# Project-MONAI/GenerativeModels

Hardware: AMD Instinct MI355X
Metric: 3D volumes/sec (DDIM 50-step sample, 1x128^3) (higher is better)
Workload: dtype bf16; 1 GPU; C2: 3D DiffusionModelUNet(64,128,256; 2 res blocks; mid-block attention 1 head x 256) DDIM-50 sampling of 1x1x128^3 volumes, 1 volume per GPU per step; inference_steps=50, parallelism=1 independent replicas (batch-sharded, no data-path collective), hip_graph=False, self_launched=False

## Files before the change

### generativemodels_amd/csrc/conv_dma.hip

```cpp
#include "conv_dma_shared.h"
#include <type_traits>

#ifdef GM_CONV_TIMELINE
#define TL_STAMP(k)                                                                                                              \
  do {                                                                                                                           \
    if ((p.debug_flags & 4096) && threadIdx.x == 0 && tl_on)                                                                            \
      reinterpret_cast<unsigned long long*>(p.kpartial)[(long long)blockIdx.x * 64 + (k)] = __builtin_readcyclecounter();        \
  } while (0)
#else
#define TL_STAMP(k)
#endif
#ifndef GM_DMA_PART
#define GM_DMA_PART (-1)
#endif
#define DMA_PART(k) (GM_DMA_PART == -1 || GM_DMA_PART == (k))
static __device__ __attribute__((aligned(64))) unsigned int gm_zero_row[16] = {0};

template <typename T, int NW, int MF, int S, int MINW, int KS = 3, int NFR_ = 4, bool PRE = false>
__global__ __launch_bounds__(64 * NW, MINW) void conv_dma_kernel(const GmConvDesc p, const unsigned phase_wgs, const unsigned phase_sleeps) {
  constexpr int BK = ConvTraits<T>::BK;
  constexpr int VECW = ConvTraits<T>::VECW;
  constexpr int NT = 64 * NW;
  constexpr int NFR = NFR_, G = KS == 3 ? 3 : 2, RING = KS == 3 ? 3 : 4;
  static_assert(KS == 3 || (KS == 2 && S == 1 && (NW == 8 || NW == 4)), "the sub-pixel variant is stride 1, 8 waves x 32 or 4 waves x 64 voxels");
  static_assert(NW * MF * 16 == 512 || NW * MF * 16 == (S == 1 ? 256 : 128), "waves x fragments cover the tile");
  constexpr int TH = 4, TW = 16, BM = NW * MF * 16, TD = BM / (TH * TW);
  constexpr int NPW = KS == 2 ? 2 : 1;
  constexpr int PD = S * (TD - 1) + KS, PH = S * (TH - 1) + KS, PW = S * (TW - 1) + KS + (NPW - 1);
  constexpr int EW = TW + 1;
  constexpr int PLANE = ((PH * PW + 15) / 16) * 16;
  constexpr int PROWS = PD * PLANE;
  constexpr int PPIECES = PROWS / 16;
  constexpr int PPW = (PPIECES + NW - 1) / NW;
  constexpr int BN = 16 * NFR;
  constexpr int WROWS = G * BN;
  constexpr bool WGEN = NFR != 4 || (KS == 2 && NW == 4);
  constexpr int PATCH_BYTES = PROWS * DMA_ROWB;
  constexpr int WBUF_BYTES = WROWS * DMA_ROWB;
  constexpr int PVT_OFF = PATCH_BYTES + (KS == 2 ? 36864 : RING * WBUF_BYTES) + 512;
  constexpr int NGROUPS = KS * KS * KS / G * NPW;
  constexpr int WPW = WGEN ? WROWS / 16 / NW : (KS == 2 ? 1 : (NW == 8 ? 2 : (NW == 4 ? 3 : 1)));
  static_assert(!WGEN || (S == 1 && (WROWS / 16) % NW == 0), "general panel distribution: whole pieces per wave");
  static_assert(WROWS == (KS == 3 ? 3 : 2) * BN, "G taps per weight panel");
  static_assert(NGROUPS % RING == 0, "the ring slot of a group is a compile-time constant");
#ifdef GM_CONV_LDS_EPILOGUE
  constexpr bool DIRECT_W = false;
#else
  constexpr bool DIRECT_W = NFR == 4 && KS == 3;
#endif

  extern __shared__ __attribute__((aligned(1024))) char smem[];
  const unsigned lds0 = (unsigned)(uintptr_t)smem;

  const int tid = threadIdx.x;
  const int lane = tid & 63;
  const int wave = __builtin_amdgcn_readfirstlane(tid >> 6);
  const int l15 = lane & 15, q = lane >> 4;
  if (blockIdx.x < phase_wgs) {
    const unsigned tg = __builtin_amdgcn_s_getreg((3 << 11) | (16 << 6) | 4);
    if (tg & 1) {
      for (unsigned k = phase_sleeps; k > 0; --k) __builtin_amdgcn_s_sleep(16);
    }
  }

  const int Dt = KS == 2 ? p.Ds : p.Do, Ht = KS == 2 ? p.Hs : p.Ho, Wt = KS == 2 ? p.Ws : p.Wo;
  const int ntd = (Dt + TD - 1) / TD, nth = (Ht + TH - 1) / TH, ntw = (Wt + TW - 1) / TW;
  const int ncb = (p.Cout + BN - 1) / BN;
  const int ksplit = (KS == 3 && S == 1 && p.kpartial && p.ksplit > 1) ? p.ksplit : 1;
  int Dv = p.Ds, Hv = p.Hs, Wv = p.Ws;
  if (p.in_mode == 1) { Dv *= p.fd; Hv *= p.fh; Wv *= p.fw; }
  const int nchunks = p.Cin / BK;
  const int cout_pad = (p.Cout + 15) & ~15;
  const int cps = ksplit > 1 ? (nchunks + ksplit - 1) / ksplit : nchunks;

  const unsigned nwork = (unsigned)p.N * ntd * nth * ntw * ncb * (KS == 2 ? 4u : 1u) * (unsigned)ksplit;
  const unsigned xcd = blockIdx.x & 7, gx = (gridDim.x >> 3) + (xcd < (gridDim.x & 7) ? 1u : 0u);
  const unsigned q8 = nwork >> 3, r8 = nwork & 7, cx = q8 + (xcd < r8 ? 1u : 0u), sx = xcd < r8 ? xcd * (q8 + 1) : r8 * (q8 + 1) + (xcd - r8) * q8;
  unsigned pos = blockIdx.x >> 3;
  if (pos >= cx) return;
#ifdef GM_CONV_TIMELINE
  const unsigned tl_pos = pos + gx < cx ? pos + gx : pos;
#endif

  struct Tile { int cb, par, n, td_i, th_i, tw_i, ks; };
  auto decode = [&](unsigned wi) __attribute__((always_inline)) {
    Tile t;
    unsigned b = wi;
    t.ks = 0;
    if (ksplit > 1) {
      const unsigned tiles_all = nwork / (unsigned)ksplit;
      t.ks = (int)(b / tiles_all);
      b -= (unsigned)t.ks * tiles_all;
    }
    t.cb = b % ncb; b /= ncb;
    t.par = 0;
    if (KS == 2) { t.par = b & 3; b >>= 2; }
    t.tw_i = b % ntw; b /= ntw;
    t.th_i = b % nth; b /= nth;
    t.td_i = b % ntd; b /= ntd;
    t.n = b;
    return t;
  };

  const char* zero = reinterpret_cast<const char*>(gm_zero_row);
  const char* xbase = reinterpret_cast<const char*>(p.x);
  int psw = 0;
#pragma unroll
  for (int j = 0; j < PPW; ++j) {
    const int row = 16 * (wave + NW * j) + (lane >> 2);
    const int rr = row % PLANE;
    psw |= dma_swz(rr % PW) << (2 * j);
  }
  int pvox[PPW];
  constexpr bool PVOX_LDS = KS == 2 && NW == 4;
  int* pvt = reinterpret_cast<int*>(smem + PVT_OFF) + threadIdx.x;
  if (PVOX_LDS) pvt[PPW * NT] = psw;
  auto place_patch = [&](const Tile& t) __attribute__((always_inline)) {
    KDesc& pk = cold_desc();
    const int ud0 = t.td_i * TD * S - (KS == 2 ? 1 - ((t.par >> 1) & 1) : pk.pd), uh0 = t.th_i * TH * S - (KS == 2 ? 1 - (t.par & 1) : pk.ph),
              uw0 = t.tw_i * TW * S - (KS == 2 ? 1 : pk.pw);
    OPAQUE_LANE(lane_p);
#pragma unroll
    for (int j = 0; j < PPW; ++j) {
      const int row = 16 * (wave + NW * j) + (lane_p >> 2);
      const int pa = row / PLANE, rr = row - pa * PLANE;
      const int pb = rr / PW, lc = rr - pb * PW;
      const int pc = S == 1 ? lc : (lc < EW ? 2 * lc : 2 * (lc - EW) + 1);
      int ud = ud0 + pa, uh = uh0 + pb, uw = uw0 + pc;
      const bool ok = (row < PROWS) & (rr < PH * PW) & (ud >= 0) & (ud < Dv) & (uh >= 0) & (uh < Hv) & (uw >= 0) & (uw < Wv);
      if (pk.in_mode == 1) { ud /= pk.fd; uh /= pk.fh; uw /= pk.fw; }
      const int pvj = ok ? ((t.n * pk.Ds + ud) * pk.Hs + uh) * pk.Ws + uw : -1;
      if (PVOX_LDS) pvt[j * NT] = pvj; else pvox[j] = pvj;
    }
  };
  const long long xrowb = p.x_ld * (long long)sizeof(T);
  const char* x2base = reinterpret_cast<const char*>(p.x2);
  const long long x2rowb = p.x2_ld * (long long)sizeof(T);
  const int nchunks0 = p.x2 ? p.cin_split / BK : nchunks;
  auto issue_patch = [&](int chunk) __attribute__((always_inline)) {
#ifdef GM_CONV_ABLATE
    if (p.debug_flags & 1024) return;
#endif
    const bool second = chunk >= nchunks0;
    const char* cbase = second ? x2base + (long long)(chunk - nchunks0) * (BK * (int)sizeof(T)) : xbase + (long long)chunk * (BK * (int)sizeof(T));
    const long long rowb = second ? x2rowb : xrowb;
#pragma unroll
    for (int j = 0; j < PPW; ++j) {
      if (wave + NW * j < PPIECES) {
        int pv = PVOX_LDS ? pvt[j * NT] : pvox[j];
        asm volatile("" : "+v"(pv));
        int ps = PVOX_LDS ? pvt[PPW * NT] : psw;
        if (PVOX_LDS) asm volatile("" : "+v"(ps));
        const char* src = pv >= 0 ? cbase + pv * rowb + (((lane & 3) ^ ((ps >> (2 * j)) & 3)) << 4) : zero + ((lane & 3) << 4);
        dma16(src, lds0 + (unsigned)(16 * (wave + NW * j)) * DMA_ROWB);
      }
    }
  };

  Tile cur = decode(sx + pos);
  const Tile stride = decode(gx);
  place_patch(cur);
  if (min(nchunks, cur.ks * cps) < nchunks) issue_patch(min(nchunks, cur.ks * cps));

  constexpr bool pre = PRE;
  float sc[VECW], sh[VECW];
  auto load_affine = [&](int chunk) __attribute__((always_inline)) {
    const int c0 = chunk * BK + (lane & 3) * VECW;
    const float* ps = p.pre_scale + (long long)cur.n * p.Cin + c0;
    const float* ph = p.pre_shift + (long long)cur.n * p.Cin + c0;
#pragma unroll
    for (int i = 0; i < VECW; i += 4) {
      const float4 a = *reinterpret_cast<const float4*>(ps + i), b = *reinterpret_cast<const float4*>(ph + i);
      sc[i] = a.x; sc[i + 1] = a.y; sc[i + 2] = a.z; sc[i + 3] = a.w;
      sh[i] = b.x; sh[i + 1] = b.y; sh[i + 2] = b.z; sh[i + 3] = b.w;
    }
  };
  auto transform_patch = [&]() __attribute__((always_inline)) {
#pragma unroll
    for (int j = 0; j < PPW; ++j) {
      if (wave + NW * j < PPIECES && pvox[j] >= 0) {
        char* a = smem + (16 * (wave + NW * j) + (lane >> 2)) * DMA_ROWB + (((lane & 3) ^ ((psw >> (2 * j)) & 3)) << 4);
        float v[VECW];
        Vec16<T>::unpack(*reinterpret_cast<const uint4*>(a), v);
#pragma unroll
        for (int i = 0; i < VECW; ++i) v[i] = v[i] * sc[i] + sh[i];
        conv_act_vec(v, p.pre_act, sizeof(T) == 4);
        *reinterpret_cast<uint4*>(a) = Vec16<T>::pack(v);
      }
    }
    asm volatile("s_waitcnt lgkmcnt(0)" ::: "memory");
  };


  const char* wbase = nullptr;
  int wsrc[WPW];
  auto place_weights = [&](const Tile& t) __attribute__((always_inline)) {
    KDesc& pk = cold_desc();
    wbase = reinterpret_cast<const char*>(pk.w) + (long long)(t.par * NPW) * nchunks * (KS * KS * KS) * cout_pad * DMA_ROWB;
    OPAQUE_LANE(lane_w);
#pragma unroll
    for (int h = 0; h < WPW; ++h) {
      const int row = WGEN ? 16 * (wave + NW * h) + (lane_w >> 2)
                    : KS == 2 ? 16 * wave + (lane_w >> 2)
                              : NW == 8 ? (h == 0 ? 16 * wave + (lane_w >> 2) : 128 + 8 * wave + ((lane_w & 31) >> 2))
                                        : (NW == 4 ? 16 * (wave + NW * h) + (lane_w >> 2) : 16 * (wave < 12 ? wave : 0) + (lane_w >> 2));
      const int u = row / BN, col = row % BN;
      const int co = t.cb * BN + (DIRECT_W ? direct_col_chan<T>(col) : col);
      wsrc[h] = co < cout_pad ? ((u * cout_pad + co) * DMA_ROWB + (((lane_w & 3) ^ dma_swz(row)) << 4)) : -1;
    }
  };
  auto issue_w_pieces = [&](int t, int buf, int h0, int h1) __attribute__((always_inline)) {
#ifdef GM_CONV_ABLATE
    if (p.debug_flags & 512) return;
#endif
    const char* panel = KS == 2 ? wbase + ((long long)((t & 7) >> 2) * nchunks * 8 + (long long)(t >> 3) * 8 + 2 * (t & 3)) * cout_pad * DMA_ROWB
                                : wbase + (long long)t * G * cout_pad * DMA_ROWB;
    const unsigned dst = lds0 + PATCH_BYTES + (unsigned)buf * WBUF_BYTES;
#pragma unroll
    for (int h = h0; h < h1; ++h) {
      const char* src = wsrc[h] >= 0 ? panel + wsrc[h] : zero + ((lane & 3) << 4);
      if (WGEN) {
        dma16(src, dst + (unsigned)(16 * (wave + NW * h)) * DMA_ROWB);
      } else if (KS == 2) {
        dma16(src, dst + (unsigned)(16 * wave) * DMA_ROWB);
      } else if (NW == 8) {
        if (h == 0) dma16(src, dst + (unsigned)(16 * wave) * DMA_ROWB);
        else if (lane < 32) dma16(src, dst + (unsigned)(128 + 8 * wave) * DMA_ROWB);
      } else if (NW == 16) {
        if (wave < 12) dma16(src, dst + (unsigned)(16 * wave) * DMA_ROWB);
      } else {
        dma16(src, dst + (unsigned)(16 * (wave + NW * h)) * DMA_ROWB);
      }
    }
  };
  auto issue_w = [&](int t, int buf) __attribute__((always_inline)) { issue_w_pieces(t, buf, 0, WPW); };


  constexpr int SCRATCH_WAVE = MF * 16 * 144, SCRATCH_BYTES = NW * SCRATCH_WAVE;
  constexpr int RING_BYTES = KS == 2 ? (RING * WBUF_BYTES > 36864 ? RING * WBUF_BYTES : 36864) : RING * WBUF_BYTES;
  constexpr bool EARLY = SCRATCH_BYTES <= RING_BYTES;
  constexpr int SCRATCH_OFF = EARLY ? PATCH_BYTES : 0;
  static_assert(EARLY || SCRATCH_BYTES <= PATCH_BYTES + RING_BYTES, "the transpose scratch fits under the addend vector");
  static_assert(BN * 8 <= SCRATCH_WAVE, "a wave's statistic partials fit into its scratch block");
  static_assert(PVT_OFF == PATCH_BYTES + RING_BYTES + 512, "the placement table follows the addend vector");
  float* addv = reinterpret_cast<float*>(smem + PATCH_BYTES + RING_BYTES);
#ifdef GM_CONV_LDS_EPILOGUE
  constexpr bool DIRECT = false;
#else
  constexpr bool DIRECT = NFR == 4 && KS == 3;
#endif
  constexpr int EPASSES = (NFR * 16 * (int)sizeof(T) + 127) / 128;
  constexpr int CH_PER_PASS = 128 / (int)sizeof(T);
  static_assert(EPASSES <= 4, "at most 4 epilogue passes (128 output channels in fp32)");

  for (;;) {
#ifdef GM_CONV_TIMELINE
    const bool tl_on = pos == tl_pos;
#endif
    TL_STAMP(0);
    const int c_begin = min(nchunks, cur.ks * cps), c_end = min(nchunks, c_begin + cps);
    const int total = (c_end - c_begin) * NGROUPS;
    const int od0 = cur.td_i * TD, oh0 = cur.th_i * TH, ow0 = cur.tw_i * TW;
    TL_STAMP(1);
    place_weights(cur);
    if (total > 0) {
      issue_w(c_begin * NGROUPS, 0);
      if (total > 1) issue_w(c_begin * NGROUPS + 1, 1);
      if (pre) load_affine(c_begin);
    }
    float addend = 0.f;
    KDesc& pa = cold_desc();
    OPAQUE_LANE(lane_a);
    const int tid_a = wave * 64 + lane_a;
    if (tid_a < BN) {
      const int co = cur.cb * BN + tid_a;
      if (co < pa.Cout) {
        if (pa.bias) addend += pa.bias[co];
        if (pa.skip_bias) addend += pa.skip_bias[co];
        if (pa.rowvec) addend += pa.rowvec[(long long)cur.n * pa.rowvec_bstride + co];
      }
    }
    TL_STAMP(55);
    constexpr int HK = S * (MF - 1) + KS;
    static_assert(MF <= 4 && (4 % MF) == 0, "a wave's fragments stay inside one 4-row tile plane");
    OPAQUE_LANE(lane_t);
    const int l15t = lane_t & 15, qt = lane_t >> 4;
    constexpr int NXA = KS + NPW - 1;
    int xa[NXA];
    {
      const int m0 = wave * MF * 16 + l15t;
      const int a = m0 >> 6, bb0 = (m0 >> 4) & 3, c = m0 & 15;
#pragma unroll
      for (int kw = 0; kw < NXA; ++kw) {
        const int col = S == 1 ? c + kw : (kw == 1 ? EW + c : c + (kw >> 1));
        xa[kw] = (S * a * PLANE + S * bb0 * PW + col) * DMA_ROWB + ((qt ^ dma_swz(col)) << 4);
      }
    }
    const int wa0 = PATCH_BYTES + l15t * DMA_ROWB + ((qt ^ dma_swz(l15t)) << 4);
#define XADDR(hk, kw) (xa[kw] + (hk) * (PW * DMA_ROWB))
#define WADDR(nf) (wa0 + (nf) * (16 * DMA_ROWB))
    f32x4_t accs[NPW][NFR][MF];
#pragma unroll
    for (int pw = 0; pw < NPW; ++pw)
#pragma unroll
      for (int nf = 0; nf < NFR; ++nf)
#pragma unroll
        for (int mf = 0; mf < MF; ++mf) accs[pw][nf][mf] = (f32x4_t){0.f, 0.f, 0.f, 0.f};
    f32x4_t (&acc)[NFR][MF] = accs[0];
    if (tid_a < BN) addv[tid_a] = addend;
    TL_STAMP(56);
    if (total > 0) {
      dma_wait<0>();
      if (pre) transform_patch();
    }
    __builtin_amdgcn_s_barrier();
#ifdef GM_CONV_TIMELINE
    if (p.debug_flags & 2048) {
      const unsigned tg = __builtin_amdgcn_s_getreg((3 << 11) | (16 << 6) | 4);
      if (tg & 1) {
        for (int k = (p.debug_flags >> 16) & 255; k > 0; --k) __builtin_amdgcn_s_sleep(1);
      }
    }
#endif
    TL_STAMP(2);

    for (int chunk = c_begin; chunk < c_end; ++chunk) {
      const bool last_chunk = chunk + 1 == c_end;
      constexpr int NH = NFR / 4;
      constexpr bool PIPE2 = NH == 1 && !PRE && (KS == 2 || S == 2 || MINW == 2);
      if constexpr (PIPE2) {
        uint4 xf[2][MF], wf[2][4];
        auto read_tap = [&](int g, int u, int set) __attribute__((always_inline)) {
          const int tap = (KS == 2 ? g % 4 : g) * G + u;
          const int kd = tap / (KS * KS), kh = (tap / KS) % KS, kw = tap % KS + (KS == 2 ? g / 4 : 0);
#pragma unroll
          for (int nf = 0; nf < 4; ++nf)
            wf[set][nf] = *reinterpret_cast<const uint4*>(smem + WADDR(nf) + (g % RING) * WBUF_BYTES + u * (BN * DMA_ROWB));
#pragma unroll
          for (int mf = 0; mf < MF; ++mf)
            xf[set][mf] = *reinterpret_cast<const uint4*>(smem + XADDR(S * mf + kh, kw) + kd * (PLANE * DMA_ROWB));
        };
        auto mma_tap_pw = [&](int set, int pw) __attribute__((always_inline)) {
#pragma unroll
          for (int nf = 0; nf < 4; ++nf)
#pragma unroll
            for (int mf = 0; mf < MF; ++mf) Mma<T>::run(wf[set][nf], xf[set][mf], accs[pw][nf][mf]);
        };
#define mma_tap(set) mma_tap_pw(set, KS == 2 ? g / 4 : 0)
        constexpr int NMMA = MF * 4 * (sizeof(T) == 2 ? 1 : 4), NRD = MF + 4;
        static_assert(G == 3 || G == 2, "taps per panel");
#ifdef GM_CONV_EARLY_BARRIER
#pragma unroll
        for (int g = 0; g < NGROUPS; ++g) {
          const int t = chunk * NGROUPS + g;
          const int X = (g * G) & 1, Y = X ^ 1;
          const int LASTSET = (g * G + G - 1) & 1, NEXTSET = ((g + 1) * G) & 1;
          if (g == 0) read_tap(0, 0, X);
          read_tap(g, 1, Y);
          mma_tap(X);
          if (g == 0) __builtin_amdgcn_sched_group_barrier(0x100, 2 * NRD, 0);
          else __builtin_amdgcn_sched_group_barrier(0x100, NRD, 0);
          __builtin_amdgcn_sched_group_barrier(0x008, NMMA, 0);
          dma_wait<0>();
          __builtin_amdgcn_s_barrier();
#ifdef GM_CONV_DMA_INTERLEAVE
          const bool want_w = g < NGROUPS - 2 || !last_chunk;
          if (G == 3) {
            read_tap(g, 2, X);
#pragma unroll
            for (int nf = 0; nf < 4; ++nf) {
#pragma unroll
              for (int mf = 0; mf < MF; ++mf) Mma<T>::run(wf[Y][nf], xf[Y][mf], acc[nf][mf]);
              if (want_w && nf < WPW) issue_w_pieces(t + 2, (g + 2) % RING, nf, nf + 1);
            }
            if (want_w && WPW > 4) issue_w_pieces(t + 2, (g + 2) % RING, 4, WPW);
          } else if (want_w) {
            issue_w(t + 2, (g + 2) % RING);
          }
#else
          if (g < NGROUPS - 2 || !last_chunk) issue_w(t + 2, (g + 2) % RING);
          if (G == 3) {
            read_tap(g, 2, X);
            mma_tap(Y);
            __builtin_amdgcn_sched_group_barrier(0x100, NRD, 0);
            __builtin_amdgcn_sched_group_barrier(0x008, NMMA, 0);
          }
#endif
          if (g == NGROUPS - 1) {
            if (!last_chunk) {
              asm volatile("s_waitcnt lgkmcnt(0)" ::: "memory");
              __builtin_amdgcn_s_barrier();
              issue_patch(chunk + 1);
              if (pre) load_affine(chunk + 1);
              dma_wait<0>();
              if (pre) transform_patch();
              __builtin_amdgcn_s_barrier();
            }
          } else {
            read_tap(g + 1, 0, NEXTSET);
          }
          mma_tap(LASTSET);
          if (g < NGROUPS - 1) {
            __builtin_amdgcn_sched_group_barrier(0x100, NRD, 0);
            __builtin_amdgcn_sched_group_barrier(0x008, NMMA, 0);
          }
          if (chunk - c_begin < 5) TL_STAMP(3 + (chunk - c_begin) * 10 + g);
        }
#else
#pragma unroll
        for (int g = 0; g < NGROUPS; ++g) {
          const int t = chunk * NGROUPS + g;
          const int X = (g * G) & 1, Y = X ^ 1;
          const int LASTSET = (g * G + G - 1) & 1, NEXTSET = ((g + 1) * G) & 1;
          if (g == 0) read_tap(0, 0, X);
          read_tap(g, 1, Y);
          mma_tap(X);
          if (g == 0) __builtin_amdgcn_sched_group_barrier(0x100, 2 * NRD, 0);
          else __builtin_amdgcn_sched_group_barrier(0x100, NRD, 0);
          __builtin_amdgcn_sched_group_barrier(0x008, NMMA, 0);
          if (g < NGROUPS - 2 || !last_chunk) issue_w(t + 2, (g + 2) % RING);
          if (G == 3) {
            read_tap(g, 2, X);
            mma_tap(Y);
            __builtin_amdgcn_sched_group_barrier(0x100, NRD, 0);
            __builtin_amdgcn_sched_group_barrier(0x008, NMMA, 0);
          }
          if (g == NGROUPS - 1) {
            if (!last_chunk) {
              asm volatile("s_waitcnt lgkmcnt(0)" ::: "memory");
              __builtin_amdgcn_s_barrier();
              issue_patch(chunk + 1);
              if (pre) load_affine(chunk + 1);
              dma_wait<0>();
              if (pre) transform_patch();
              __builtin_amdgcn_s_barrier();
            }
          } else {
            if ((g < NGROUPS - 2 || !last_chunk) && (NW != 16 || wave < 12)) dma_wait<WPW>(); else dma_wait<0>();
            __builtin_amdgcn_s_barrier();
            read_tap(g + 1, 0, NEXTSET);
          }
          mma_tap(LASTSET);
          if (g < NGROUPS - 1) {
            __builtin_amdgcn_sched_group_barrier(0x100, NRD, 0);
            __builtin_amdgcn_sched_group_barrier(0x008, NMMA, 0);
          }
          if (chunk - c_begin < 5) TL_STAMP(3 + (chunk - c_begin) * 10 + g);
        }
#endif
      } else {
#pragma unroll
      for (int g = 0; g < NGROUPS; ++g) {
        const int t = chunk * NGROUPS + g;
        if (g < NGROUPS - 2 || !last_chunk) issue_w(t + 2, (g + 2) % RING);
        constexpr int NSTEPS = G * NH;
        uint4 xf[MF], wf[4];
        auto read_step = [&](int st) __attribute__((always_inline)) {
          const int u = st / NH, hf = st % NH;
          const int tap = g * G + u;
          const int kd = tap / (KS * KS), kh = (tap / KS) % KS, kw = tap % KS;
#pragma unroll
          for (int nf = 0; nf < 4; ++nf)
            wf[nf] = *reinterpret_cast<const uint4*>(smem + WADDR(nf) + hf * (64 * DMA_ROWB) + (g % RING) * WBUF_BYTES + u * (BN * DMA_ROWB));
          if (hf == 0) {
#pragma unroll
            for (int mf = 0; mf < MF; ++mf)
              xf[mf] = *reinterpret_cast<const uint4*>(smem + XADDR(S * mf + kh, kw) + kd * (PLANE * DMA_ROWB));
          }
        };
        auto mma_step = [&](int st) __attribute__((always_inline)) {
          const int hf = st % NH;
#pragma unroll
          for (int nf = 0; nf < 4; ++nf)
#pragma unroll
            for (int mf = 0; mf < MF; ++mf) Mma<T>::run(wf[nf], xf[mf], acc[hf * 4 + nf][mf]);
        };
        constexpr int NMMA = MF * 4 * (sizeof(T) == 2 ? 1 : 4);
#pragma unroll
        for (int st = 0; st < NSTEPS - 1; ++st) {
          read_step(st);
          mma_step(st);
          if (st % NH == 0) __builtin_amdgcn_sched_group_barrier(0x100, MF + 4, 0);
          else __builtin_amdgcn_sched_group_barrier(0x100, 4, 0);
          __builtin_amdgcn_sched_group_barrier(0x008, NMMA, 0);
        }
        read_step(NSTEPS - 1);
        if (g == NGROUPS - 1) {
          if (!last_chunk) {
            asm volatile("s_waitcnt lgkmcnt(0)" ::: "memory");
            __builtin_amdgcn_s_barrier();
            issue_patch(chunk + 1);
            if (pre) load_affine(chunk + 1);
            dma_wait<0>();
            if (pre) transform_patch();
            __builtin_amdgcn_s_barrier();
          }
        } else {
          if ((g < NGROUPS - 2 || !last_chunk) && (NW != 16 || wave < 12)) dma_wait<WPW>(); else dma_wait<0>();
          __builtin_amdgcn_s_barrier();
        }
        mma_step(NSTEPS - 1);
        if (chunk - c_begin < 5) TL_STAMP(3 + (chunk - c_begin) * 10 + g);
      }
      }
    }
  TL_STAMP(60);

    const EpTile et = {cur.n, od0, oh0, ow0, cur.cb * BN, cur.par * NPW};
    const bool partial = KS == 3 && S == 1 && ksplit > 1;
    EpRows<MF * 2> rowsP[NPW];
    EpRows<MF * 2>& rows0 = rowsP[0];
    OPAQUE_LANE(lane_e);
    constexpr int NST = 16 / VECW;
    constexpr bool RES_AHEAD = sizeof(T) == 2;
    bool d_direct = false, d_lane_ok = false;
    int d_yoff = 0, d_roff = 0;
    if constexpr (DIRECT) {
      KDesc& pd = cold_desc();
      d_direct = pd.post_act == 0 && !partial;
      if (d_direct) {
        const int l15e = lane_e & 15, qe = lane_e >> 4;
        const int Wl = KS == 2 ? pd.Ws : pd.Wo;
        const int lw = KS == 2 ? 2 * l15e : l15e;
        d_yoff = lw * (int)(pd.y_ld * (long long)sizeof(T)) + 16 * qe;
        d_roff = lw * (int)(pd.res_ld * (long long)sizeof(T)) + 16 * qe;
        d_lane_ok = ow0 + l15e < Wl;
#pragma unroll
        for (int it = 0; it < MF * 2; ++it) rows0.rv[it] = make_uint4(0u, 0u, 0u, 0u);
        if (RES_AHEAD && pd.res) {
          const int Dl = KS == 2 ? pd.Ds : pd.Do, Hl = KS == 2 ? pd.Hs : pd.Ho;
#pragma unroll
          for (int mf = 0; mf < MF; ++mf) {
            const int line = wave * MF + mf;
            const int od = od0 + (line >> 2), oh = oh0 + (line & 3);
            if (od < Dl && oh < Hl) {
              const long long vrow = KS == 2 ? (((long long)cur.n * pd.Do + 2 * od + ((cur.par >> 2) & 1)) * pd.Ho + 2 * oh + ((cur.par >> 1) & 1)) * pd.Wo + 2 * ow0 + (cur.par & 1)
                                             : (((long long)cur.n * pd.Do + od) * pd.Ho + oh) * pd.Wo + ow0;
              const char* rrow = reinterpret_cast<const char*>(pd.res) + (vrow * pd.res_ld + cur.cb * BN) * (long long)sizeof(T);
#pragma unroll
              for (int st = 0; st < NST; ++st) {
                const int cfirst = cur.cb * BN + (64 * st + 16 * qe) / (int)sizeof(T);
                if (d_lane_ok && cfirst < pd.Cout) rows0.rv[(mf * NST + st) % (MF * 2)] = *reinterpret_cast<const uint4*>(rrow + (unsigned)(d_roff + 64 * st));
              }
            }
          }
        }
      }
    }
    if (!partial && !d_direct) {
#pragma unroll
      for (int pw = 0; pw < NPW; ++pw) {
        const EpTile etp = {et.n, et.od0, et.oh0, et.ow0, et.co_base, et.par + pw};
        dma_epilogue_rows<T, MF, KS, 0>(cold_desc(), etp, wave * MF, lane_e, rowsP[pw]);
      }
    }

    KDesc& ps = cold_desc();
    if (ps.skip_x[0] && cur.ks == ksplit - 1) {
      const int nsc0 = ps.skip_cin[0] / BK, nsc = nsc0 + (ps.skip_x[1] ? ps.skip_cin[1] / BK : 0);
      OPAQUE_LANE(lane_k);
      const int pswz = ((lane_k & 3) ^ dma_swz(lane_k >> 2)) << 4;
      int svox[MF];
  #pragma unroll
      for (int h = 0; h < MF; ++h) {
        const int m = wave * (MF * 16) + h * 16 + (lane_k >> 2);
        const int od = od0 + (m >> 6), oh = oh0 + ((m >> 4) & 3), ow = ow0 + (m & 15);
        svox[h] = (od < ps.Do && oh < ps.Ho && ow < ps.Wo) ? ((cur.n * ps.Do + od) * ps.Ho + oh) * ps.Wo + ow : -1;
      }
      const int wpiece = WGEN ? wave : (wave & 3);
      const int wcol = wpiece * 16 + (lane_k >> 2);
      const int wco = cur.cb * BN + (DIRECT_W ? direct_col_chan<T>(wcol) : wcol);
      const int wswz = ((lane_k & 3) ^ dma_swz(wcol)) << 4;
      int caddr[MF];
  #pragma unroll
      for (int mf = 0; mf < MF; ++mf) {
        const int m = (wave * MF + mf) * 16 + (lane_k & 15);
        caddr[mf] = m * DMA_ROWB + (((lane_k >> 4) ^ dma_swz(m)) << 4);
      }
      const char* wsk = reinterpret_cast<const char*>(ps.skip_w);
      for (int sc0 = 0; sc0 < nsc; sc0 += 2) {
        asm volatile("s_waitcnt vmcnt(0) lgkmcnt(0)" ::: "memory");
        __builtin_amdgcn_s_barrier();
  #pragma unroll
        for (int j = 0; j < 2; ++j) {
          const int sc = sc0 + j;
          if (sc < nsc) {
            const int part = sc >= nsc0 ? 1 : 0, cip = sc - (part ? nsc0 : 0);
            const char* xb = reinterpret_cast<const char*>(ps.skip_x[part]) + (long long)cip * (BK * (int)sizeof(T)) + pswz;
            const long long rowb = ps.skip_ld[part] * (long long)sizeof(T);
  #pragma unroll
            for (int h = 0; h < MF; ++h) {
              const char* src = svox[h] >= 0 ? xb + svox[h] * rowb : zero + ((lane_k & 3) << 4);
              dma16(src, lds0 + (unsigned)(j * BM + wave * (MF * 16) + h * 16) * DMA_ROWB);
            }
            if (WGEN || NW == 4 || (wave >> 2) == j) {
              const char* src = wco < cout_pad ? wsk + ((long long)sc * cout_pad + wco) * DMA_ROWB + wswz : zero + ((lane_k & 3) << 4);
              dma16(src, lds0 + PATCH_BYTES + (unsigned)(j * BN + wpiece * 16) * DMA_ROWB);
            }
          }
        }
        asm volatile("s_waitcnt vmcnt(0)" ::: "memory");
        __builtin_amdgcn_s_barrier();
  #pragma unroll
        for (int j = 0; j < 2; ++j) {
          if (sc0 + j < nsc) {
            uint4 xf[MF], wf[4];
  #pragma unroll
            for (int mf = 0; mf < MF; ++mf) xf[mf] = *reinterpret_cast<const uint4*>(smem + caddr[mf] + j * (BM * DMA_ROWB));
  #pragma unroll
            for (int hf = 0; hf < NFR / 4; ++hf) {
  #pragma unroll
              for (int nf = 0; nf < 4; ++nf)
                wf[nf] = *reinterpret_cast<const uint4*>(smem + WADDR(nf) + hf * (64 * DMA_ROWB) + j * (BN * DMA_ROWB));
  #pragma unroll
              for (int nf = 0; nf < 4; ++nf)
  #pragma unroll
                for (int mf = 0; mf < MF; ++mf) Mma<T>::run(wf[nf], xf[mf], acc[hf * 4 + nf][mf]);
            }
          }
        }
      }
    }


    TL_STAMP(61);
    const bool has_next = pos + gx < cx;
    const bool has_next_early = !DIRECT || has_next || partial;
    if (has_next_early) {
      asm volatile("s_waitcnt lgkmcnt(0)" ::: "memory");
      __builtin_amdgcn_s_barrier();
    }
    Tile nxt = cur;
    if (has_next) {
      if (ksplit > 1) {
        nxt = decode(sx + pos + gx);
      } else {
        int c;
        nxt.cb = cur.cb + stride.cb; c = nxt.cb >= ncb ? 1 : 0; nxt.cb -= c ? ncb : 0;
        if (KS == 2) { nxt.par = cur.par + stride.par + c; c = nxt.par >> 2; nxt.par &= 3; }
        nxt.tw_i = cur.tw_i + stride.tw_i + c; c = nxt.tw_i >= ntw ? 1 : 0; nxt.tw_i -= c ? ntw : 0;
        nxt.th_i = cur.th_i + stride.th_i + c; c = nxt.th_i >= nth ? 1 : 0; nxt.th_i -= c ? nth : 0;
        nxt.td_i = cur.td_i + stride.td_i + c; c = nxt.td_i >= ntd ? 1 : 0; nxt.td_i -= c ? ntd : 0;
        nxt.n = cur.n + stride.n + c;
      }
      place_patch(nxt);
      if (EARLY && min(nchunks, nxt.ks * cps) < nchunks) issue_patch(min(nchunks, nxt.ks * cps));
    }
    TL_STAMP(57);
    KDesc& pe = cold_desc();
    if (KS == 3 && S == 1 && ksplit > 1) {
      const long long nv = (long long)pe.N * pe.Do * pe.Ho * pe.Wo;
      float* part = pe.kpartial + (long long)cur.ks * nv * pe.Cout;
  #pragma unroll
      for (int mf = 0; mf < MF; ++mf) {
        const int m = (wave * MF + mf) * 16 + (lane_e & 15);
        const int od = od0 + (m >> 6), oh = oh0 + ((m >> 4) & 3), ow = ow0 + (m & 15);
        if (od < pe.Do && oh < pe.Ho && ow < pe.Wo) {
          float* row = part + ((((long long)cur.n * pe.Do + od) * pe.Ho + oh) * pe.Wo + ow) * pe.Cout;
  #pragma unroll
          for (int nf = 0; nf < NFR; ++nf) {
            const int co = cur.cb * BN + (DIRECT ? direct_chan<T>(nf, lane_e >> 4, 0) : nf * 16 + (lane_e >> 4) * 4);
            if (co < pe.Cout)
              *reinterpret_cast<float4*>(row + co) = make_float4(acc[nf][mf][0], acc[nf][mf][1], acc[nf][mf][2], acc[nf][mf][3]);
          }
        }
      }
    } else {

#ifdef GM_CONV_ABLATE
    if (!(pe.debug_flags & 256)) {
#endif
    if (DIRECT && d_direct) {
      const int qe = lane_e >> 4;
      typedef float f32x2_t __attribute__((ext_vector_type(2)));
      f32x2_t ds[NST][VECW / 2], dq[NST][VECW / 2];
#pragma unroll
      for (int st = 0; st < NST; ++st)
#pragma unroll
        for (int i = 0; i < VECW / 2; ++i) { ds[st][i] = (f32x2_t){0.f, 0.f}; dq[st][i] = (f32x2_t){0.f, 0.f}; }
      const int Dl = KS == 2 ? pe.Ds : pe.Do, Hl = KS == 2 ? pe.Hs : pe.Ho, Wl = KS == 2 ? pe.Ws : pe.Wo;
      const bool has_res = pe.res != nullptr, has_stats = pe.stats != nullptr;
      const bool full = od0 + TD <= Dl && oh0 + TH <= Hl && ow0 + TW <= Wl && (cur.cb + 1) * BN <= pe.Cout;
      bool ok_st[NST];
#pragma unroll
      for (int st = 0; st < NST; ++st) ok_st[st] = d_lane_ok && cur.cb * BN + (64 * st + 16 * qe) / (int)sizeof(T) < pe.Cout;
      f32x2_t addl[NST][VECW / 2];
#pragma unroll
      for (int st = 0; st < NST; ++st)
#pragma unroll
        for (int i = 0; i < VECW; i += 4) {
          const float4 a = *reinterpret_cast<const float4*>(addv + (64 * st) / (int)sizeof(T) + qe * VECW + i);
          addl[st][i / 2] = (f32x2_t){a.x, a.y};
          addl[st][i / 2 + 1] = (f32x2_t){a.z, a.w};
        }
      auto direct_stores = [&](auto RESc, auto FULLc) __attribute__((always_inline)) {
        constexpr bool RES = decltype(RESc)::value, FULL = decltype(FULLc)::value;
#pragma unroll
        for (int mf = 0; mf < MF; ++mf) {
          const int line = wave * MF + mf;
          const int od = od0 + (line >> 2), oh = oh0 + (line & 3);
          const bool row_ok = FULL || (od < Dl && oh < Hl);
          const long long vrow = KS == 2 ? (((long long)cur.n * pe.Do + 2 * od + ((cur.par >> 2) & 1)) * pe.Ho + 2 * oh + ((cur.par >> 1) & 1)) * pe.Wo + 2 * ow0 + (cur.par & 1)
                                         : (((long long)cur.n * pe.Do + od) * pe.Ho + oh) * pe.Wo + ow0;
          char* yrow = reinterpret_cast<char*>(pe.y) + (vrow * pe.y_ld + cur.cb * BN) * (long long)sizeof(T);
          const char* rrow = reinterpret_cast<const char*>(pe.res) + (vrow * pe.res_ld + cur.cb * BN) * (long long)sizeof(T);
#pragma unroll
          for (int st = 0; st < NST; ++st) {
            const bool ok = FULL || (row_ok && ok_st[st]);
            f32x2_t o[VECW / 2];
#pragma unroll
            for (int i = 0; i < VECW / 2; ++i) {
              const f32x4_t c = acc[st * (VECW / 4) + (i >> 1)][mf];
              o[i] = (i & 1 ? (f32x2_t){c[2], c[3]} : (f32x2_t){c[0], c[1]}) + addl[st][i];
            }
            uint32_t w[4];
            auto pack4 = [&]() __attribute__((always_inline)) {
              if (sizeof(T) == 2) {
#pragma unroll
                for (int i = 0; i < VECW / 2; ++i) w[i] = pack_bf16x2(o[i][0], o[i][1]);
              } else {
                w[0] = __float_as_uint(o[0][0]); w[1] = __float_as_uint(o[0][1]); w[2] = __float_as_uint(o[1][0]); w[3] = __float_as_uint(o[1][1]);
              }
            };
            auto unpack4 = [&](const uint32_t (&u)[4], f32x2_t (&v)[VECW / 2]) __attribute__((always_inline)) {
              if (sizeof(T) == 2) {
#pragma unroll
                for (int i = 0; i < VECW / 2; ++i) v[i] = (f32x2_t){__uint_as_float(u[i] << 16), __uint_as_float(u[i] & 0xffff0000u)};
              } else {
                v[0] = (f32x2_t){__uint_as_float(u[0]), __uint_as_float(u[1])};
                v[1] = (f32x2_t){__uint_as_float(u[2]), __uint_as_float(u[3])};
              }
            };
            pack4();
            if (RES) {
              uint4 rv = RES_AHEAD ? rows0.rv[(mf * NST + st) % (MF * 2)] : make_uint4(0u, 0u, 0u, 0u);
              if (!RES_AHEAD && ok) rv = *reinterpret_cast<const uint4*>(rrow + (unsigned)(d_roff + 64 * st));
              const uint32_t ru[4] = {rv.x, rv.y, rv.z, rv.w};
              f32x2_t r[VECW / 2];
              unpack4(w, o);
              unpack4(ru, r);
#pragma unroll
              for (int i = 0; i < VECW / 2; ++i) o[i] += r[i];
              pack4();
            }
            if (ok) *reinterpret_cast<uint4*>(yrow + (unsigned)(d_yoff + 64 * st)) = make_uint4(w[0], w[1], w[2], w[3]);
            if (!FULL) {
#pragma unroll
              for (int i = 0; i < 4; ++i) w[i] = ok ? w[i] : 0u;
            }
            unpack4(w, o);
#pragma unroll
            for (int i = 0; i < VECW / 2; ++i) {
              ds[st][i] += o[i];
              dq[st][i] = __builtin_elementwise_fma(o[i], o[i], dq[st][i]);
            }
          }
        }
      };
      if (has_res) {
        if (full) direct_stores(std::true_type{}, std::true_type{}); else direct_stores(std::true_type{}, std::false_type{});
      } else {
        if (full) direct_stores(std::false_type{}, std::true_type{}); else direct_stores(std::false_type{}, std::false_type{});
      }
      TL_STAMP(62);
      if (has_stats) {
        constexpr int DSTEPS = NW <= 4 ? 0 : (NW == 8 ? 1 : 2), WL = 16 >> DSTEPS, WSCR = RING_BYTES / NW;
        static_assert(4 * WL * 144 <= WSCR && BN * 8 <= WSCR, "a wave's statistic rows fit into its share of the weight ring");
        OPAQUE_LANE(lane_s);
        if (DSTEPS >= 1) {
#pragma unroll
          for (int st = 0; st < NST; ++st)
#pragma unroll
            for (int i = 0; i < VECW; ++i) { ds[st][i / 2][i & 1] += dpp_row_ror8(ds[st][i / 2][i & 1]); dq[st][i / 2][i & 1] += dpp_row_ror8(dq[st][i / 2][i & 1]); }
        }
        if (DSTEPS >= 2) {
#pragma unroll
          for (int st = 0; st < NST; ++st)
#pragma unroll
            for (int i = 0; i < VECW; ++i) { ds[st][i / 2][i & 1] += dpp_row_ror4(ds[st][i / 2][i & 1]); dq[st][i / 2][i & 1] += dpp_row_ror4(dq[st][i / 2][i & 1]); }
        }
        if (!has_next_early) {
          asm volatile("s_waitcnt lgkmcnt(0)" ::: "memory");
          __builtin_amdgcn_s_barrier();
        }
        char* wscr = smem + PATCH_BYTES + (size_t)wave * WSCR;
        const int l15s = lane_s & 15, qs = lane_s >> 4;
        if (l15s < WL) {
          char* rowp = wscr + (qs * WL + l15s) * 144;
#pragma unroll
          for (int st = 0; st < NST; ++st)
#pragma unroll
            for (int i = 0; i < VECW; i += 2)
              *reinterpret_cast<float4*>(rowp + (st * VECW + i) * 8) = make_float4(ds[st][i / 2][0], dq[st][i / 2][0], ds[st][i / 2][1], dq[st][i / 2][1]);
        }
        __builtin_amdgcn_fence(__ATOMIC_RELEASE, "wavefront");
        __builtin_amdgcn_wave_barrier();
        __builtin_amdgcn_fence(__ATOMIC_ACQUIRE, "wavefront");
        const int bch = lane_s * (int)sizeof(T);
        const char* colp = wscr + (((bch & 63) >> 4) * WL) * 144 + ((bch >> 6) * VECW + (bch & 15) / (int)sizeof(T)) * 8;
        float sa = 0.f, sb = 0.f;
#pragma unroll
        for (int w = 0; w < WL; ++w) {
          const float2 v = *reinterpret_cast<const float2*>(colp + w * 144);
          sa += v.x;
          sb += v.y;
        }
        __builtin_amdgcn_fence(__ATOMIC_RELEASE, "wavefront");
        __builtin_amdgcn_wave_barrier();
        __builtin_amdgcn_fence(__ATOMIC_ACQUIRE, "wavefront");
        *reinterpret_cast<float2*>(wscr + lane_s * 8) = make_float2(sa, sb);
        __syncthreads();
        const int ch = wave * 64 + lane_s;
        if (ch < BN) {
          double a = 0.0, b2 = 0.0;
#pragma unroll
          for (int w = 0; w < NW; ++w) {
            const float2 v = *reinterpret_cast<const float2*>(smem + PATCH_BYTES + w * WSCR + ch * 8);
            a += (double)v.x;
            b2 += (double)v.y;
          }
          const int co = cur.cb * BN + ch;
          if (co < pe.Cout) {
            const long long slot = ((long long)(cur.td_i * nth + cur.th_i) * ntw + cur.tw_i) * (KS == 2 ? 8 : 1) + cur.par;
            double* dst = pe.stats + ((slot * pe.N + cur.n) * pe.Cout + co) * 2;
            *reinterpret_cast<double2*>(dst) = make_double2(a, b2);
          }
        }
      }
    } else {
    if (DIRECT && !has_next_early) {
      asm volatile("s_waitcnt lgkmcnt(0)" ::: "memory");
      __builtin_amdgcn_s_barrier();
    }
#pragma unroll
    for (int pw = 0; pw < NPW; ++pw) {
    const EpTile etp = {et.n, et.od0, et.oh0, et.ow0, et.co_base, et.par + pw};
    if (pw > 0) {
      asm volatile("s_waitcnt lgkmcnt(0)" ::: "memory");
      __builtin_amdgcn_s_barrier();
    }
    float st_s[EPASSES][VECW], st_q[EPASSES][VECW];
#pragma unroll
    for (int e = 0; e < EPASSES; ++e)
#pragma unroll
      for (int i = 0; i < VECW; ++i) { st_s[e][i] = 0.f; st_q[e][i] = 0.f; }
    char* scratch = smem + SCRATCH_OFF + (size_t)wave * SCRATCH_WAVE;
    dma_epilogue_pass<T, MF, NFR, KS, 0, DIRECT>(pe, accs[pw], scratch, addv, etp, wave * MF, lane_e, rowsP[pw], st_s, st_q);
    if constexpr (EPASSES > 1) {
      EpRows<MF * 2> rows;
      dma_epilogue_rows<T, MF, KS, 1>(pe, etp, wave * MF, lane_e, rows);
      dma_epilogue_pass<T, MF, NFR, KS, 1, DIRECT>(pe, accs[pw], scratch, addv, etp, wave * MF, lane_e, rows, st_s, st_q);
    }
    if constexpr (EPASSES > 2) {
      EpRows<MF * 2> rows;
      dma_epilogue_rows<T, MF, KS, 2>(pe, etp, wave * MF, lane_e, rows);
      dma_epilogue_pass<T, MF, NFR, KS, 2, DIRECT>(pe, accs[pw], scratch, addv, etp, wave * MF, lane_e, rows, st_s, st_q);
    }
    if constexpr (EPASSES > 3) {
      EpRows<MF * 2> rows;
      dma_epilogue_rows<T, MF, KS, 3>(pe, etp, wave * MF, lane_e, rows);
      dma_epilogue_pass<T, MF, NFR, KS, 3, DIRECT>(pe, accs[pw], scratch, addv, etp, wave * MF, lane_e, rows, st_s, st_q);
    }
    TL_STAMP(62);
    if (pe.stats) {
      OPAQUE_LANE(lane_s);
      float ra[EPASSES][VECW], rb[EPASSES][VECW];
#pragma unroll
      for (int e = 0; e < EPASSES; ++e)
#pragma unroll
        for (int i = 0; i < VECW; ++i) { ra[e][i] = wave_segment_sum(st_s[e][i]); rb[e][i] = wave_segment_sum(st_q[e][i]); }
      if (lane_s < 8) {
        float* part = reinterpret_cast<float*>(scratch);
#pragma unroll
        for (int e = 0; e < EPASSES; ++e)
#pragma unroll
          for (int i = 0; i < VECW; i += 2)
            *reinterpret_cast<float4*>(part + 2 * (e * CH_PER_PASS + lane_s * VECW + i)) = make_float4(ra[e][i], rb[e][i], ra[e][i + 1], rb[e][i + 1]);
      }
      __syncthreads();
      const int ch = wave * 64 + lane_s;
      if (ch < BN) {
        double a = 0.0, b2 = 0.0;
#pragma unroll
        for (int w = 0; w < NW; ++w) {
          const float2 v = *reinterpret_cast<const float2*>(smem + SCRATCH_OFF + w * SCRATCH_WAVE + ch * 8);
          a += (double)v.x;
          b2 += (double)v.y;
        }
        const int co = cur.cb * BN + ch;
        if (co < pe.Cout) {
          const long long slot = ((long long)(cur.td_i * nth + cur.th_i) * ntw + cur.tw_i) * (KS == 2 ? 8 : 1) + etp.par;
          double* dst = pe.stats + ((slot * pe.N + cur.n) * pe.Cout + co) * 2;
          *reinterpret_cast<double2*>(dst) = make_double2(a, b2);
        }
      }
    }
    }
    }
#ifdef GM_CONV_ABLATE
    }
#endif
    }
    TL_STAMP(63);
    if (!has_next) break;
    asm volatile("s_waitcnt lgkmcnt(0)" ::: "memory");
    __builtin_amdgcn_s_barrier();
    if (!EARLY && min(nchunks, nxt.ks * cps) < nchunks) issue_patch(min(nchunks, nxt.ks * cps));
    cur = nxt;
    pos += gx;
  }
}

#undef mma_tap
#undef XADDR
#undef WADDR

extern "C" int gm_conv_sn_eligible(const GmConvDesc* d);
extern "C" int gm_conv_sn_launch(const GmConvDesc* dp, unsigned nblocks, void* stream);
extern "C" int gm_conv_sk_eligible(const GmConvDesc* d);
extern "C" int gm_conv_sk_launch(const GmConvDesc* dp, unsigned nblocks, void* stream);

#if DMA_PART(0)
extern "C" long long gm_conv_dma_lds_bytes(int variant) {
  const long long addv = 512;
  if (variant == 4) return 5LL * 96 * DMA_ROWB + 36864 + addv + 256LL * 9 * 4;
  if (variant == 5) return 10LL * 112 * DMA_ROWB + 3LL * 384 * DMA_ROWB + addv;
  const long long plane = variant == 2 ? 304 : 112, planes = variant == 1 ? 6 : (variant == 2 ? 5 : 10);
  return planes * plane * DMA_ROWB + 3LL * 192 * DMA_ROWB + addv;
}

#endif
#if DMA_PART(0)
int gm_dma_grid_cap = 0;
extern "C" void gm_conv_dma_set_persistent(int max_work_groups) { gm_dma_grid_cap = max_work_groups; }

int gm_dma_phase_skew = 0;
extern "C" void gm_conv_dma_set_phase_skew(int cycles) { gm_dma_phase_skew = cycles; }
#else
extern int gm_dma_grid_cap, gm_dma_phase_skew;
#endif
#define g_dma_grid_cap gm_dma_grid_cap
#define g_dma_phase_skew gm_dma_phase_skew
extern "C" long long gm_conv_dma_lds_bytes(int variant);
extern "C" int gm_conv_dma_variant(int cfg);
static int dma_device_cus() {
  static int cus = 0;
  if (cus == 0) {
    int dev = 0, n = 0;
    if (hipGetDevice(&dev) != hipSuccess || hipDeviceGetAttribute(&n, hipDeviceAttributeMultiprocessorCount, dev) != hipSuccess || n <= 0) n = 256;
    cus = n;
  }
  return cus;
}

static unsigned dma_grid(unsigned nwork, long long lds_bytes, int by_waves, bool splitk) {
  if (splitk || g_dma_grid_cap == 0) return nwork;
  long long cap = g_dma_grid_cap;
  if (cap < 0) {
    const int cus = dma_device_cus();
    long long per_cu = (160LL * 1024) / lds_bytes;
    if (per_cu > by_waves) per_cu = by_waves;
    if (per_cu < 1) per_cu = 1;
    cap = per_cu * cus;
  }
  if (cap < 8) cap = 8;
  return nwork < (unsigned)cap ? nwork : (unsigned)cap;
}

#if DMA_PART(0)
extern "C" int gm_conv_dma_variant(int cfg) { return cfg == 17 ? 4 : (cfg == 15 ? 2 : (cfg == 16 || cfg == 18 ? 3 : (cfg == 19 ? 5 : 1))); }

extern "C" int gm_conv_dma_eligible(const GmConvDesc* d) {
  if (d->cfg == 21 || d->cfg == 22) return 0;
  if (d->cfg == 24 || d->cfg == 25) return gm_conv_sn_eligible(d);
  const int bk = d->dtype == GM_F32 ? 16 : 32;
  const int vecw = d->dtype == GM_F32 ? 4 : 8;
  const int s = d->cfg == 15 ? 2 : 1;
  if (d->cfg == 17) {
    return d->in_mode == 3 && d->kd == 2 && d->kh == 2 && d->kw == 2 && d->sd == 1 && d->sh == 1 && d->sw == 1 && d->dd == 1 && d->dh == 1 &&
           d->dw == 1 && d->Do == 2 * d->Ds && d->Ho == 2 * d->Hs && d->Wo == 2 * d->Ws && d->Cin % bk == 0 && d->x_ld % vecw == 0 &&
           (reinterpret_cast<uintptr_t>(d->x) & 15) == 0 && d->pre_scale == nullptr && d->pre_act == 0 && d->x2 == nullptr && d->ltd == 2 && d->lth == 2 &&
           d->ltw == 4 && d->Cout % vecw == 0 && d->y_ld % vecw == 0 && (reinterpret_cast<uintptr_t>(d->y) & 15) == 0 &&
           (!d->res || (d->res_ld % vecw == 0 && (reinterpret_cast<uintptr_t>(d->res) & 15) == 0)) && !d->skip_x[0] &&
           (long long)d->N * d->Do * d->Ho * d->Wo < (1LL << 31);
  }
  if (d->in_mode == 3) return 0;
  return d->kd == 3 && d->kh == 3 && d->kw == 3 && d->sd == s && d->sh == s && d->sw == s && d->dd == 1 && d->dh == 1 && d->dw == 1 &&
         (d->in_mode == 0 || (d->in_mode == 1 && s == 1)) && d->Cin % bk == 0 && d->x_ld % vecw == 0 &&
         (reinterpret_cast<uintptr_t>(d->x) & 15) == 0 &&
         ((d->pre_stats[0] == nullptr &&
           ((d->pre_scale == nullptr && d->pre_shift == nullptr && d->pre_act == 0) ||
            (s == 1 && d->pre_scale != nullptr && d->pre_shift != nullptr && (reinterpret_cast<uintptr_t>(d->pre_scale) & 15) == 0 &&
             (reinterpret_cast<uintptr_t>(d->pre_shift) & 15) == 0 && (d->Cin % 4) == 0))) ||
          (d->pre_stats[0] != nullptr && d->cfg == 11 && gm_conv_sk_eligible(d))) &&
         (d->x2 == nullptr || (d->cin_split > 0 && d->cin_split < d->Cin && d->cin_split % bk == 0 && d->x2_ld % vecw == 0 &&
                               (reinterpret_cast<uintptr_t>(d->x2) & 15) == 0)) &&
         d->ltd == (d->cfg == 16 || d->cfg == 18 || d->cfg == 19 ? 3 : (s == 1 ? 2 : 1)) && d->lth == 2 &&
         d->ltw == 4 && d->Cout % vecw == 0 && d->y_ld % vecw == 0 && (reinterpret_cast<uintptr_t>(d->y) & 15) == 0 &&
         (!d->res || (d->res_ld % vecw == 0 && (reinterpret_cast<uintptr_t>(d->res) & 15) == 0)) &&
         (long long)d->N * d->Ds * d->Hs * d->Ws < (1LL << 31) && (long long)d->N * d->Do * d->Ho * d->Wo < (1LL << 31) &&
         (!d->skip_x[0] ||
          (d->skip_w && d->skip_cin[0] > 0 && d->skip_cin[0] % bk == 0 && d->skip_ld[0] % vecw == 0 &&
           (reinterpret_cast<uintptr_t>(d->skip_x[0]) & 15) == 0 &&
           (!d->skip_x[1] || (d->skip_cin[1] > 0 && d->skip_cin[1] % bk == 0 && d->skip_ld[1] % vecw == 0 &&
                              (reinterpret_cast<uintptr_t>(d->skip_x[1]) & 15) == 0))));
}

#endif
template <typename T, int NW, int MF, int S, int MINW, int KS = 3, int NFR = 4, bool PRE = false>
static void launch_dma(const GmConvDesc& d, unsigned nblocks, hipStream_t st) {
  static bool attr_set = false;
  auto kern = conv_dma_kernel<T, NW, MF, S, MINW, KS, NFR, PRE>;
  if (!attr_set) {
    hipError_t e = hipFuncSetAttribute(reinterpret_cast<const void*>(kern), hipFuncAttributeMaxDynamicSharedMemorySize, 160 * 1024);
    if (e != hipSuccess) (void)hipGetLastError();
    attr_set = true;
  }
  const long long lds = gm_conv_dma_lds_bytes(gm_conv_dma_variant(d.cfg));
  const bool splitk = d.ksplit > 1 && d.kpartial != nullptr;
  constexpr int BY_WAVES = MINW * 4 / NW >= 1 ? MINW * 4 / NW : 1;
  const unsigned grid = dma_grid(nblocks, lds, BY_WAVES, splitk);
  long long per_cu = (160LL * 1024) / lds;
  if (per_cu > BY_WAVES) per_cu = BY_WAVES;
  const unsigned resident = (unsigned)(per_cu * dma_device_cus());
  unsigned phase_wgs = 0, phase_sleeps = 0;
  if (per_cu >= 2 && !splitk && g_dma_phase_skew != 0 && nblocks >= 2 * resident) {
    long long cycles = g_dma_phase_skew;
    if (cycles < 0) {
      const long long chunks = d.Cin / (d.dtype == GM_F32 ? 16 : 32), taps = KS * KS * KS;
      const long long mfma_cycles = chunks * taps * (MF * NFR) * (d.dtype == GM_F32 ? 4 * 8 : 16);
      const long long waves_per_simd = per_cu * NW / 4 > 0 ? per_cu * NW / 4 : 1;
      cycles = (18000 + waves_per_simd * mfma_cycles) / 2;
    }
    phase_wgs = resident;
    phase_sleeps = (unsigned)((cycles + 512) / 1024);
    if (phase_sleeps == 0) phase_wgs = 0;
  }
  kern<<<dim3(grid), 64 * NW, (size_t)lds, st>>>(d, phase_wgs, phase_sleeps);
}

#define DMA_BY_DTYPE(...)                                                                    \
  do {                                                                                       \
    if (d.dtype == GM_F32) { using T = float; __VA_ARGS__; return 0; }                       \
    if (d.dtype == GM_BF16) { using T = bf16_raw; __VA_ARGS__; return 0; }                   \
    return -2;                                                                               \
  } while (0)
extern "C" int gm_conv_dma_launch_part0(const GmConvDesc* dp, unsigned nblocks, void* stream);
extern "C" int gm_conv_dma_launch_part1(const GmConvDesc* dp, unsigned nblocks, void* stream);
extern "C" int gm_conv_dma_launch_part2(const GmConvDesc* dp, unsigned nblocks, void* stream);
extern "C" int gm_conv_dma_launch_part3(const GmConvDesc* dp, unsigned nblocks, void* stream);
extern "C" int gm_conv_dma_launch_part4(const GmConvDesc* dp, unsigned nblocks, void* stream);
#if DMA_PART(0)
extern "C" int gm_conv_dma_launch_part0(const GmConvDesc* dp, unsigned nblocks, void* stream) {
  const GmConvDesc& d = *dp; hipStream_t st = (hipStream_t)stream;
  const bool pre = d.pre_scale != nullptr;
  DMA_BY_DTYPE(if (pre) launch_dma<T, 8, 2, 1, 4, 3, 4, true>(d, nblocks, st); else launch_dma<T, 8, 2, 1, 4>(d, nblocks, st));
}
#endif
#if DMA_PART(1)
extern "C" int gm_conv_dma_launch_part1(const GmConvDesc* dp, unsigned nblocks, void* stream) {
  const GmConvDesc& d = *dp; hipStream_t st = (hipStream_t)stream;
  const bool pre = d.pre_scale != nullptr;
  DMA_BY_DTYPE(if (pre) launch_dma<T, 4, 4, 1, 2, 3, 4, true>(d, nblocks, st); else launch_dma<T, 4, 4, 1, 2>(d, nblocks, st));
}
#endif
#if DMA_PART(2)
extern "C" int gm_conv_dma_launch_part2(const GmConvDesc* dp, unsigned nblocks, void* stream) {
  const GmConvDesc& d = *dp; hipStream_t st = (hipStream_t)stream;
  if (d.cfg == 17) DMA_BY_DTYPE((launch_dma<T, 4, 4, 1, 2, 2>(d, nblocks, st)));
  DMA_BY_DTYPE((launch_dma<T, 8, 1, 2, 2>(d, nblocks, st)));
}
#endif
#if DMA_PART(3)
extern "C" int gm_conv_dma_launch_part3(const GmConvDesc* dp, unsigned nblocks, void* stream) {
  const GmConvDesc& d = *dp; hipStream_t st = (hipStream_t)stream;
  const bool pre = d.pre_scale != nullptr;
  if (d.cfg == 18) DMA_BY_DTYPE(if (pre) launch_dma<T, 8, 4, 1, 2, 3, 4, true>(d, nblocks, st); else launch_dma<T, 8, 4, 1, 2>(d, nblocks, st));
  DMA_BY_DTYPE(if (pre) launch_dma<T, 16, 2, 1, 4, 3, 4, true>(d, nblocks, st); else launch_dma<T, 16, 2, 1, 4>(d, nblocks, st));
}
#endif
#if DMA_PART(4)
extern "C" int gm_conv_dma_launch_part4(const GmConvDesc* dp, unsigned nblocks, void* stream) {
  const GmConvDesc& d = *dp; hipStream_t st = (hipStream_t)stream;
  const bool pre = d.pre_scale != nullptr;
  DMA_BY_DTYPE(if (pre) launch_dma<T, 8, 4, 1, 2, 3, 8, true>(d, nblocks, st); else launch_dma<T, 8, 4, 1, 2, 3, 8>(d, nblocks, st));
}
#endif

#if DMA_PART(0)
extern "C" int gm_conv_dma_launch(const GmConvDesc* dp, unsigned nblocks, void* stream) {
  if (dp->cfg == 24 || dp->cfg == 25) return gm_conv_sn_launch(dp, nblocks, stream);
  if (gm_conv_sk_eligible(dp)) return gm_conv_sk_launch(dp, nblocks, stream);
  switch (dp->cfg) {
    case 14: return gm_conv_dma_launch_part1(dp, nblocks, stream);
    case 15: case 17: return gm_conv_dma_launch_part2(dp, nblocks, stream);
    case 16: case 18: return gm_conv_dma_launch_part3(dp, nblocks, stream);
    case 19: return gm_conv_dma_launch_part4(dp, nblocks, stream);
    default: return gm_conv_dma_launch_part0(dp, nblocks, stream);
  }
}
#endif
```

Baseline: 1.371 volumes/s.

## Pipeline the fused skip-connection GEMM with a multi-stage DMA ring

Replaces the fused 1x1 skip-projection loop, which loaded two channel chunks and then drained all DMA before computing, with a 2- or 3-stage ring buffer carved from the existing operand LDS area. Loads for later chunks are issued while the current chunk's MMAs run, with per-stage partial waits instead of full vmcnt(0) drains. Weight panels are redistributed so each wave issues one panel instruction. The path is also restricted to KS==3 kernels, and the slot-reuse ordering adds a risk of synchronisation hazards.

```diff
diff --git a/generativemodels_amd/csrc/conv_dma.hip b/generativemodels_amd/csrc/conv_dma.hip
--- a/generativemodels_amd/csrc/conv_dma.hip
+++ b/generativemodels_amd/csrc/conv_dma.hip
@@ -556,8 +556,14 @@
     }
 
     KDesc& ps = cold_desc();
-    if (ps.skip_x[0] && cur.ks == ksplit - 1) {
+    if (KS == 3 && ps.skip_x[0] && cur.ks == ksplit - 1) {
       const int nsc0 = ps.skip_cin[0] / BK, nsc = nsc0 + (ps.skip_x[1] ? ps.skip_cin[1] / BK : 0);
+      constexpr int SXB = BM * DMA_ROWB, SPB = BN * DMA_ROWB;
+      constexpr int NS = 3 * (SXB + SPB) <= PATCH_BYTES + RING_BYTES ? 3 : 2;
+      constexpr int SW_OFF = NS * SXB;
+      constexpr int SWR = BN / NW;
+      static_assert(NS * (SXB + SPB) <= PATCH_BYTES + RING_BYTES, "the stages fit into the operand area: no LDS is added");
+      static_assert(SWR * NW == BN && (SWR == 16 || SWR == 8 || SWR == 4), "one panel instruction per wave");
       OPAQUE_LANE(lane_k);
       const int pswz = ((lane_k & 3) ^ dma_swz(lane_k >> 2)) << 4;
       int svox[MF];
@@ -567,10 +573,9 @@
         const int od = od0 + (m >> 6), oh = oh0 + ((m >> 4) & 3), ow = ow0 + (m & 15);
         svox[h] = (od < ps.Do && oh < ps.Ho && ow < ps.Wo) ? ((cur.n * ps.Do + od) * ps.Ho + oh) * ps.Wo + ow : -1;
       }
-      const int wpiece = WGEN ? wave : (wave & 3);
-      const int wcol = wpiece * 16 + (lane_k >> 2);
-      const int wco = cur.cb * BN + (DIRECT_W ? direct_col_chan<T>(wcol) : wcol);
-      const int wswz = ((lane_k & 3) ^ dma_swz(wcol)) << 4;
+      const int wrow = wave * SWR + (lane_k >> 2);
+      const int wco = cur.cb * BN + (DIRECT_W ? direct_col_chan<T>(wrow) : wrow);
+      const int wswz = ((lane_k & 3) ^ dma_swz(wrow)) << 4;
       int caddr[MF];
   #pragma unroll
       for (int mf = 0; mf < MF; ++mf) {
@@ -578,47 +583,57 @@
         caddr[mf] = m * DMA_ROWB + (((lane_k >> 4) ^ dma_swz(m)) << 4);
       }
       const char* wsk = reinterpret_cast<const char*>(ps.skip_w);
-      for (int sc0 = 0; sc0 < nsc; sc0 += 2) {
-        asm volatile("s_waitcnt vmcnt(0) lgkmcnt(0)" ::: "memory");
+      auto issue_sx = [&](int sc, int slot) __attribute__((always_inline)) {
+        const int part = sc >= nsc0 ? 1 : 0, cip = sc - (part ? nsc0 : 0);
+        const char* xb = reinterpret_cast<const char*>(ps.skip_x[part]) + (long long)cip * (BK * (int)sizeof(T)) + pswz;
+        const long long rowb = ps.skip_ld[part] * (long long)sizeof(T);
+  #pragma unroll
+        for (int h = 0; h < MF; ++h) {
+          const char* src = svox[h] >= 0 ? xb + svox[h] * rowb : zero + ((lane_k & 3) << 4);
+          dma16(src, lds0 + (unsigned)(slot * SXB) + (unsigned)(wave * (MF * 16) + h * 16) * DMA_ROWB);
+        }
+      };
+      auto issue_sw = [&](int sc, int slot) __attribute__((always_inline)) {
+        const char* src = wco < cout_pad ? wsk + ((long long)sc * cout_pad + wco) * DMA_ROWB + wswz : zero + ((lane_k & 3) << 4);
+        if (SWR == 16 || lane_k < 4 * SWR) dma16(src, lds0 + (unsigned)(SW_OFF + slot * SPB) + (unsigned)(wave * SWR) * DMA_ROWB);
+      };
+      asm volatile("s_waitcnt lgkmcnt(0)" ::: "memory");
+      __builtin_amdgcn_s_barrier();
+  #pragma unroll
+      for (int k = 0; k < NS; ++k) {
+        if (k < nsc) {
+          issue_sx(k, k);
+          issue_sw(k, k);
+        }
+      }
+      int slot = 0;
+      for (int s = 0; s < nsc; ++s) {
+        const int left = nsc - 1 - s;
+        if (NS == 3) {
+          if (left >= 2) dma_wait<2 * MF + 1>(); else if (left == 1) dma_wait<MF + 1>(); else dma_wait<0>();
+        } else {
+          if (left >= 1) dma_wait<MF>(); else dma_wait<0>();
+        }
         __builtin_amdgcn_s_barrier();
+        if (s >= 1 && s - 1 + NS < nsc) issue_sw(s - 1 + NS, slot == 0 ? NS - 1 : slot - 1);
+        uint4 xf[MF], wf[4];
   #pragma unroll
-        for (int j = 0; j < 2; ++j) {
-          const int sc = sc0 + j;
-          if (sc < nsc) {
-            const int part = sc >= nsc0 ? 1 : 0, cip = sc - (part ? nsc0 : 0);
-            const char* xb = reinterpret_cast<const char*>(ps.skip_x[part]) + (long long)cip * (BK * (int)sizeof(T)) + pswz;
-            const long long rowb = ps.skip_ld[part] * (long long)sizeof(T);
+        for (int mf = 0; mf < MF; ++mf) xf[mf] = *reinterpret_cast<const uint4*>(smem + caddr[mf] + slot * SXB);
   #pragma unroll
-            for (int h = 0; h < MF; ++h) {
-              const char* src = svox[h] >= 0 ? xb + svox[h] * rowb : zero + ((lane_k & 3) << 4);
-              dma16(src, lds0 + (unsigned)(j * BM + wave * (MF * 16) + h * 16) * DMA_ROWB);
-            }
-            if (WGEN || NW == 4 || (wave >> 2) == j) {
-              const char* src = wco < cout_pad ? wsk + ((long long)sc * cout_pad + wco) * DMA_ROWB + wswz : zero + ((lane_k & 3) << 4);
-              dma16(src, lds0 + PATCH_BYTES + (unsigned)(j * BN + wpiece * 16) * DMA_ROWB);
-            }
-          }
-        }
-        asm volatile("s_waitcnt vmcnt(0)" ::: "memory");
-        __builtin_amdgcn_s_barrier();
+        for (int hf = 0; hf < NFR / 4; ++hf) {
   #pragma unroll
-        for (int j = 0; j < 2; ++j) {
-          if (sc0 + j < nsc) {
-            uint4 xf[MF], wf[4];
+          for (int nf = 0; nf < 4; ++nf)
+            wf[nf] = *reinterpret_cast<const uint4*>(smem + WADDR(nf) + hf * (64 * DMA_ROWB) + (SW_OFF - PATCH_BYTES) + slot * SPB);
+          if (hf == 0) {
+            asm volatile("s_waitcnt lgkmcnt(0)" ::: "memory");
+            if (s + NS < nsc) issue_sx(s + NS, slot);
+          }
   #pragma unroll
-            for (int mf = 0; mf < MF; ++mf) xf[mf] = *reinterpret_cast<const uint4*>(smem + caddr[mf] + j * (BM * DMA_ROWB));
+          for (int nf = 0; nf < 4; ++nf)
   #pragma unroll
-            for (int hf = 0; hf < NFR / 4; ++hf) {
-  #pragma unroll
-              for (int nf = 0; nf < 4; ++nf)
-                wf[nf] = *reinterpret_cast<const uint4*>(smem + WADDR(nf) + hf * (64 * DMA_ROWB) + j * (BN * DMA_ROWB));
-  #pragma unroll
-              for (int nf = 0; nf < 4; ++nf)
-  #pragma unroll
-                for (int mf = 0; mf < MF; ++mf) Mma<T>::run(wf[nf], xf[mf], acc[hf * 4 + nf][mf]);
-            }
-          }
-        }
+            for (int mf = 0; mf < MF; ++mf) Mma<T>::run(wf[nf], xf[mf], acc[hf * 4 + nf][mf]);
+        }
+        slot = slot + 1 == NS ? 0 : slot + 1;
       }
     }
 
```

Result: no change. 1.369 volumes/s (median of 2 runs) (-0.2%).
